# flanggut/smvs

Hardware: NVIDIA H100
Metric: Gauss-Newton Mpix-iters/sec (higher is better)
Workload: dtype f64

## Files before the change

### smvs_b200/csrc/cg.cu

```cuda
#include <algorithm>
#include <cstring>

#include "common.cuh"

namespace smvsb {

namespace {

constexpr int CG_THREADS = 256;
constexpr int CG_WARPS = CG_THREADS / 32;
constexpr int CG_QUADS = CG_THREADS / 4;
constexpr int CG_MAX_BLOCKS = 1024;
constexpr int CG_UF = 4;
constexpr int CG_SLOTS = 10;

struct CgView
{
    int n_nodes, npx;
    int grid;
    int pad;
    double err_tol;
    double const* H;
    double const* P;
    double const* g;
    uint16_t const* rowmask;
    uint32_t const* rows;
    unsigned long long const* counts;
    double* x;
    double* r;
    double* d;
    double* d2;
    double* Ad;
    double* z;
    double* partials;
    double* result;
};

struct CgArgs
{
    int n_views;
    int max_iter;
    double q_tol;
    unsigned int* sync;
    CgView v[SMVSB_MAX_BATCH];
};

struct CgState
{
    double r_dot_r, Q0, beta, alpha, tol;
    double* partials;
    int n_rows, passes, done, iters, info;
    int grid;
};

__device__ __forceinline__ void
grid_barrier (unsigned int* counter, unsigned int& epoch)
{
    __syncthreads();
    if (threadIdx.x == 0)
    {
        epoch += 1;
        unsigned int const target = epoch * gridDim.x;
        asm volatile("red.release.gpu.global.add.u32 [%0], 1;"
            :: "l"(counter) : "memory");
        unsigned int v;
        do {
            asm volatile("ld.relaxed.gpu.global.u32 %0, [%1];"
                : "=r"(v) : "l"(counter) : "memory");
        } while (v < target);
        asm volatile("ld.acquire.gpu.global.u32 %0, [%1];"
            : "=r"(v) : "l"(counter) : "memory");
    }
    __syncthreads();
}

__device__ __forceinline__ unsigned long long
policy_evict_first (void)
{
    unsigned long long pol;
    asm("createpolicy.fractional.L2::evict_first.b64 %0, 1.0;" : "=l"(pol));
    return pol;
}

__device__ __forceinline__ void
ld_stream (double const* p, double2& h01, double2& h23)
{
    unsigned long long const pol = policy_evict_first();
    asm volatile("ld.global.L1::no_allocate.L2::cache_hint.v2.f64 "
        "{%0, %1}, [%2], %3;"
        : "=d"(h01.x), "=d"(h01.y) : "l"(p), "l"(pol));
    asm volatile("ld.global.L1::no_allocate.L2::cache_hint.v2.f64 "
        "{%0, %1}, [%2], %3;"
        : "=d"(h23.x), "=d"(h23.y) : "l"(p + 2), "l"(pol));
}

__device__ __forceinline__ double2
ld_vec (double const* p)
{
    return *reinterpret_cast<double2 const*>(p);
}

__device__ __forceinline__ double2
ld_hint (double const* p, unsigned long long policy)
{
    double2 v;
    asm volatile("ld.global.L2::cache_hint.v2.f64 {%0, %1}, [%2], %3;"
        : "=d"(v.x), "=d"(v.y) : "l"(p), "l"(policy));
    return v;
}

__device__ __forceinline__ unsigned long long
policy_evict_last (void)
{
    unsigned long long pol;
    asm volatile("createpolicy.fractional.L2::evict_last.b64 %0, 1.0;"
        : "=l"(pol));
    return pol;
}

template <int NV>
__device__ __forceinline__ void
warp_flush (double (&v)[NV], double* s_red, int view)
{
#pragma unroll
    for (int j = 0; j < NV; ++j)
        for (int off = 16; off > 0; off >>= 1)
            v[j] += __shfl_down_sync(0xffffffffu, v[j], off);
    if ((threadIdx.x & 31) == 0)
    {
#pragma unroll
        for (int j = 0; j < NV; ++j)
            s_red[(view * 3 + j) * CG_WARPS + (threadIdx.x >> 5)] = v[j];
    }
}

template <int NV>
__device__ __forceinline__ void
publish (CgArgs const& a, CgState const* s_state, double const* s_red,
    int first_slot, bool init)
{
    __syncthreads();
    int const t = threadIdx.x;
    if (t < a.n_views * NV)
    {
        int const view = t / NV, j = t % NV;
        CgState const& S = s_state[view];
        if (static_cast<int>(blockIdx.x) < S.grid && (init || !S.done))
        {
            double total = 0.0;
            if (S.passes > 0)
                for (int i = 0; i < CG_WARPS; ++i)
                    total += s_red[(view * 3 + j) * CG_WARPS + i];
            S.partials[(first_slot + j) * CG_MAX_BLOCKS + blockIdx.x] = total;
        }
    }
}

template <int NV>
__device__ __forceinline__ void
all_sums (CgArgs const& a, CgState const* s_state, int first_slot,
    double* s_bcast, bool init)
{
    __syncthreads();
    int const warp = threadIdx.x >> 5, lane = threadIdx.x & 31;
    for (int pair = warp; pair < a.n_views * NV; pair += CG_WARPS)
    {
        int const view = pair / NV, j = pair % NV;
        if (!init && s_state[view].done)
            continue;
        double const* p = s_state[view].partials
            + (first_slot + j) * CG_MAX_BLOCKS;
        int const nb = s_state[view].grid;
        double v = 0.0;
        for (int base = lane; base < nb; base += 32 * 12)
        {
            double t[12];
#pragma unroll
            for (int u = 0; u < 12; ++u)
                t[u] = (base + 32 * u < nb) ? __ldcg(p + base + 32 * u) : 0.0;
#pragma unroll
            for (int u = 0; u < 12; ++u)
                if (base + 32 * u < nb)
                    v += t[u];
        }
        for (int off = 16; off > 0; off >>= 1)
            v += __shfl_down_sync(0xffffffffu, v, off);
        if (lane == 0)
            s_bcast[view * 3 + j] = v;
    }
    __syncthreads();
}

struct PlainVec
{
    double const* v;
    __device__ __forceinline__ void load (int node, double* out) const
    {
        double2 const a = *reinterpret_cast<double2 const*>(
            v + static_cast<size_t>(node) * 4);
        double2 const b = *reinterpret_cast<double2 const*>(
            v + static_cast<size_t>(node) * 4 + 2);
        out[0] = a.x; out[1] = a.y; out[2] = b.x; out[3] = b.y;
    }
};

struct DirVec
{
    double const* z;
    double const* d_old;
    double beta;
    __device__ __forceinline__ void load (int node, double* out) const
    {
        double2 const z0 = ld_vec(z + static_cast<size_t>(node) * 4);
        double2 const z1 = ld_vec(z + static_cast<size_t>(node) * 4 + 2);
        double2 const d0 = ld_vec(d_old + static_cast<size_t>(node) * 4);
        double2 const d1 = ld_vec(d_old + static_cast<size_t>(node) * 4 + 2);
        out[0] = z0.x + d0.x * beta; out[1] = z0.y + d0.y * beta;
        out[2] = z1.x + d1.x * beta; out[3] = z1.y + d1.y * beta;
    }
};

template <typename VecOp>
__device__ __forceinline__ double
spmv_row (double const* __restrict__ H, int ns, VecOp const& vec, int node,
    int rp, unsigned int mask, double* own)
{
    int const ix = node % ns, iy = node / ns;
    double const* hrow = H + static_cast<size_t>(node) * 144 + rp * 4;
    double acc = 0.0;
    own[0] = 0.0; own[1] = 0.0; own[2] = 0.0; own[3] = 0.0;
    if (mask == 0)
        return 0.0;
#pragma unroll
    for (int k = 0; k < 9; ++k)
    {
        if (!((mask >> k) & 1u))
            continue;
        int const jx = ix + (k % 3) - 1, jy = iy + (k / 3) - 1;
        int const nj = jy * ns + jx;
        double2 h01, h23;
        ld_stream(hrow + k * 16, h01, h23);
        double v[4];
        vec.load(nj, v);
        if (k == 4)
        {
            own[0] = v[0]; own[1] = v[1]; own[2] = v[2]; own[3] = v[3];
        }
        acc += h01.x * v[0];
        acc += h01.y * v[1];
        acc += h23.x * v[2];
        acc += h23.y * v[3];
    }
    return acc;
}

__device__ __forceinline__ bool
view_on (CgArgs const& a, CgState const* s_state, int v, bool init)
{
    return static_cast<int>(blockIdx.x) < s_state[v].grid
        && (init || !s_state[v].done) && s_state[v].passes > 0;
}

__device__ __forceinline__ bool
pass_row (CgView const& V, int n_rows, int pass, int& node)
{
    int const q = pass * (V.grid * CG_QUADS) + blockIdx.x * CG_QUADS
        + (threadIdx.x >> 2);
    bool const ok = q < n_rows;
    node = ok ? static_cast<int>(V.rows[q]) : 0;
    return ok;
}

template <int NV>
__global__ void __launch_bounds__(CG_THREADS, 2)
cg_kernel (CgArgs const a)
{
    unsigned long long const keep = policy_evict_last();
    __shared__ double s_red[NV * 3 * CG_WARPS];
    __shared__ double s_bcast[NV * 3];
    __shared__ CgState s_state[NV];
    __shared__ double const* s_zptr[NV];
    unsigned int epoch = 0;
    int const quad = threadIdx.x & 28;
    int const rp = threadIdx.x & 3;

    if (threadIdx.x < a.n_views)
    {
        CgView const& V = a.v[threadIdx.x];
        CgState& S = s_state[threadIdx.x];
        S.n_rows = static_cast<int>(V.counts[1]);
        int const per_pass = V.grid * CG_QUADS;
        int const passes = (S.n_rows + per_pass - 1) / per_pass;
        S.passes = ((passes + CG_UF - 1) / CG_UF) * CG_UF;
        S.done = 0; S.iters = 0; S.info = SMVSB_CG_MAX_ITERATIONS;
        S.r_dot_r = 0.0; S.Q0 = 0.0; S.beta = 0.0; S.alpha = 0.0; S.tol = 0.0;
        S.partials = V.partials;
        S.grid = V.grid;
        s_zptr[threadIdx.x] = V.z;
    }
    __syncthreads();

#pragma unroll
    for (int v = 0; v < NV; ++v)
    {
        if (v >= a.n_views || !view_on(a, s_state, v, true))
            continue;
        CgView const& V = a.v[v];
        int const n_rows = s_state[v].n_rows, passes = s_state[v].passes;
        double acc[2] = { 0.0, 0.0 };
        for (int p = 0; p < passes; ++p)
        {
            int node;
            bool const ok = pass_row(V, n_rows, p, node);
            size_t const i = static_cast<size_t>(node) * 4 + rp;
            double const gi = ok ? V.g[i] : 0.0;
            double const ri = -gi;
            double const r0 = __shfl_sync(0xffffffffu, ri, quad);
            double const r1 = __shfl_sync(0xffffffffu, ri, quad + 1);
            double const r2 = __shfl_sync(0xffffffffu, ri, quad + 2);
            double const r3 = __shfl_sync(0xffffffffu, ri, quad + 3);
            if (ok)
            {
                double const* prow = V.P + static_cast<size_t>(node) * 16
                    + rp * 4;
                double2 const p01 = *reinterpret_cast<double2 const*>(prow);
                double2 const p23 = *reinterpret_cast<double2 const*>(prow + 2);
                double const zi = p01.x * r0 + p01.y * r1 + p23.x * r2
                    + p23.y * r3;
                V.r[i] = ri;
                V.z[i] = zi;
                V.d[i] = 0.0;
                V.d2[i] = 0.0;
                V.Ad[i] = 0.0;
                acc[1] += gi * gi;
                acc[0] += zi * ri;
            }
        }
        warp_flush<2>(acc, s_red, v);
    }
    publish<2>(a, s_state, s_red, 0, true);
    grid_barrier(a.sync, epoch);
    all_sums<2>(a, s_state, 0, s_bcast, true);
    if (threadIdx.x < a.n_views)
    {
        CgState& S = s_state[threadIdx.x];
        S.r_dot_r = s_bcast[threadIdx.x * 3 + 0];
        double const gg = s_bcast[threadIdx.x * 3 + 1];
        double const et = a.v[threadIdx.x].err_tol;
        S.tol = (et < 0.0) ? sqrt(gg) * 0.01 : et;
    }
    __syncthreads();

    int iter = 1;
    int first_node[NV];
    unsigned int first_mask[NV];
#pragma unroll
    for (int v = 0; v < NV; ++v)
    {
        first_node[v] = 0;
        first_mask[v] = 0u;
        if (v < a.n_views && static_cast<int>(blockIdx.x) < s_state[v].grid)
        {
            int const quad0 = blockIdx.x * CG_QUADS + (threadIdx.x >> 2);
            if (quad0 < s_state[v].n_rows)
            {
                first_node[v] = static_cast<int>(a.v[v].rows[quad0]);
                first_mask[v] = a.v[v].rowmask[first_node[v]];
            }
        }
    }
    for (; iter < a.max_iter; ++iter)
    {
        bool const odd = (iter & 1) != 0;
        int const slot = 2 + 4 * (iter & 1);

        {
#pragma unroll
            for (int v = 0; v < NV; ++v)
            {
                if (v >= a.n_views || !view_on(a, s_state, v, false))
                    continue;
                CgView const& V = a.v[v];
                int const n_rows = s_state[v].n_rows;
                int const quads = V.grid * CG_QUADS;
                int const quad0 = blockIdx.x * CG_QUADS + (threadIdx.x >> 2);
                DirVec dir;
                dir.z = s_zptr[v];
                dir.d_old = odd ? V.d : V.d2;
                dir.beta = s_state[v].beta;
                double* d_new = odd ? V.d2 : V.d;
                double acc[1] = { 0.0 };
                int node = first_node[v];
                unsigned int mask = first_mask[v];
                for (int q = quad0; q < n_rows; q += quads)
                {
                    int const qn = q + quads;
                    int const node_next = (qn < n_rows)
                        ? static_cast<int>(V.rows[qn]) : 0;
                    unsigned int const mask_next = (qn < n_rows)
                        ? V.rowmask[node_next] : 0u;
                    double own[4];
                    size_t const i = static_cast<size_t>(node) * 4 + rp;
                    double const val = spmv_row(V.H, V.npx + 1, dir, node, rp,
                        mask, own);
                    node = node_next;
                    mask = mask_next;
                    double const di = (rp == 0) ? own[0] : (rp == 1) ? own[1]
                        : (rp == 2) ? own[2] : own[3];
                    V.Ad[i] = val;
                    d_new[i] = di;
                    acc[0] += val * di;
                }
                warp_flush<1>(acc, s_red, v);
            }
            publish<1>(a, s_state, s_red, slot, false);
        }
        grid_barrier(a.sync, epoch);
        all_sums<1>(a, s_state, slot, s_bcast, false);
        if (threadIdx.x < a.n_views && !s_state[threadIdx.x].done)
            s_state[threadIdx.x].alpha = s_state[threadIdx.x].r_dot_r
                / s_bcast[threadIdx.x * 3];
        __syncthreads();

#pragma unroll
        for (int v = 0; v < NV; ++v)
        {
            if (v >= a.n_views || !view_on(a, s_state, v, false))
                continue;
            CgView const& V = a.v[v];
            int const n_rows = s_state[v].n_rows;
            int const passes = s_state[v].passes;
            double const alpha = s_state[v].alpha;
            double const* d_new = odd ? V.d2 : V.d;
            double acc[3] = { 0.0, 0.0, 0.0 };
            int nodes[CG_UF];
            bool oks[CG_UF];
#pragma unroll
            for (int u = 0; u < CG_UF; ++u)
                oks[u] = pass_row(V, n_rows, u, nodes[u]);
            for (int p = 0; p < passes; p += CG_UF)
            {
                int nodes_next[CG_UF];
                bool oks_next[CG_UF];
#pragma unroll
                for (int u = 0; u < CG_UF; ++u)
                    oks_next[u] = pass_row(V, n_rows, p + CG_UF + u,
                        nodes_next[u]);

                double xv[CG_UF], rv[CG_UF], gv[CG_UF];
                double2 p01[CG_UF], p23[CG_UF];
#pragma unroll
                for (int u = 0; u < CG_UF; ++u)
                {
                    xv[u] = 0.0; rv[u] = 0.0; gv[u] = 0.0;
                    p01[u] = make_double2(0, 0); p23[u] = p01[u];
                    if (oks[u])
                    {
                        size_t const i = static_cast<size_t>(nodes[u]) * 4 + rp;
                        double const dn = d_new[i], ad = V.Ad[i];
                        gv[u] = V.g[i];
                        xv[u] = V.x[i]; rv[u] = V.r[i];
                        double const* prow = V.P
                            + static_cast<size_t>(nodes[u]) * 16 + rp * 4;
                        p01[u] = ld_hint(prow, keep);
                        p23[u] = ld_hint(prow + 2, keep);
                        xv[u] += dn * alpha; rv[u] -= ad * alpha;
                    }
                }
#pragma unroll
                for (int u = 0; u < CG_UF; ++u)
                {
                    double const q0 = __shfl_sync(0xffffffffu, rv[u], quad);
                    double const q1 = __shfl_sync(0xffffffffu, rv[u], quad + 1);
                    double const q2 = __shfl_sync(0xffffffffu, rv[u], quad + 2);
                    double const q3 = __shfl_sync(0xffffffffu, rv[u], quad + 3);
                    if (oks[u])
                    {
                        size_t const i = static_cast<size_t>(nodes[u]) * 4 + rp;
                        double const zi = p01[u].x * q0 + p01[u].y * q1
                            + p23[u].x * q2 + p23[u].y * q3;
                        V.x[i] = xv[u]; V.r[i] = rv[u];
                        V.z[i] = zi;
                        acc[0] += rv[u] * rv[u];
                        acc[1] += xv[u] * (rv[u] - gv[u]);
                        acc[2] += zi * rv[u];
                    }
                }
#pragma unroll
                for (int u = 0; u < CG_UF; ++u)
                {
                    nodes[u] = nodes_next[u];
                    oks[u] = oks_next[u];
                }
            }
            warp_flush<3>(acc, s_red, v);
        }
        publish<3>(a, s_state, s_red, slot + 1, false);
        grid_barrier(a.sync, epoch);
        all_sums<3>(a, s_state, slot + 1, s_bcast, false);

        if (threadIdx.x < a.n_views && !s_state[threadIdx.x].done)
        {
            CgState& S = s_state[threadIdx.x];
            double const new_rr = s_bcast[threadIdx.x * 3 + 0];
            double const xbr = s_bcast[threadIdx.x * 3 + 1];
            double const new_zr = s_bcast[threadIdx.x * 3 + 2];
            bool stop = false;
            if (new_rr < S.tol)
                stop = true;
            else
            {
                double const Q1 = -1.0 * xbr;
                double const zeta = iter * (Q1 - S.Q0) / Q1;
                if (zeta < a.q_tol)
                    stop = true;
                else
                {
                    S.Q0 = Q1;
                    S.beta = new_zr / S.r_dot_r;
                    S.r_dot_r = new_zr;
                }
            }
            if (stop)
            {
                S.done = 1;
                S.iters = iter;
                S.info = SMVSB_CG_CONVERGENCE;
            }
        }
        __syncthreads();
        bool all_done = true;
        for (int v = 0; v < a.n_views; ++v)
            all_done = all_done && (s_state[v].done != 0);
        if (all_done)
            break;
    }

    if (blockIdx.x == 0 && threadIdx.x < a.n_views)
    {
        CgState const& S = s_state[threadIdx.x];
        double* res = a.v[threadIdx.x].result;
        res[0] = S.done ? S.iters : iter;
        res[1] = S.info;
        res[2] = isnan(__ldcg(a.v[threadIdx.x].x)) ? 1.0 : 0.0;
    }
}

__global__ void __launch_bounds__(256)
cg_mark_kernel (int npx, int npy, uint8_t const* __restrict__ node_valid,
    uint8_t const* __restrict__ active, uint16_t* __restrict__ rowmask,
    uint32_t* __restrict__ block_rows, unsigned long long* __restrict__ counts)
{
    int const node = blockIdx.x * blockDim.x + threadIdx.x;
    int const ns = npx + 1;
    unsigned int m = 0;
    if (node < ns * (npy + 1) && node_valid[node] && active[node])
    {
        int const ix = node % ns, iy = node / ns;
        for (int k = 0; k < 9; ++k)
        {
            int const jx = ix + (k % 3) - 1, jy = iy + (k / 3) - 1;
            if (jx < 0 || jx > npx || jy < 0 || jy > npy)
                continue;
            int const nj = jy * ns + jx;
            if (node_valid[nj] && active[nj])
                m |= 1u << k;
        }
    }
    if (node < ns * (npy + 1))
        rowmask[node] = static_cast<uint16_t>(m);
    unsigned int const blocks = __reduce_add_sync(0xffffffffu, __popc(m));
    int const rows = __syncthreads_count(m != 0);
    if ((threadIdx.x & 31) == 0)
        atomicAdd(counts, static_cast<unsigned long long>(blocks));
    if (threadIdx.x == 0)
    {
        block_rows[blockIdx.x] = rows;
        atomicAdd(counts + 1, static_cast<unsigned long long>(rows));
    }
}

__global__ void __launch_bounds__(1024)
cg_scan_kernel (uint32_t const* __restrict__ block_rows,
    uint32_t* __restrict__ block_off, int nb)
{
    __shared__ uint32_t s_warp[32];
    __shared__ uint32_t s_carry;
    if (threadIdx.x == 0)
        s_carry = 0;
    __syncthreads();
    int const lane = threadIdx.x & 31, warp = threadIdx.x >> 5;
    for (int base = 0; base < nb; base += 1024)
    {
        int const i = base + threadIdx.x;
        uint32_t const v = (i < nb) ? block_rows[i] : 0;
        uint32_t inc = v;
        for (int o = 1; o < 32; o <<= 1)
        {
            uint32_t const u = __shfl_up_sync(0xffffffffu, inc, o);
            if (lane >= o)
                inc += u;
        }
        if (lane == 31)
            s_warp[warp] = inc;
        __syncthreads();
        if (warp == 0)
        {
            uint32_t w = s_warp[lane];
            for (int o = 1; o < 32; o <<= 1)
            {
                uint32_t const u = __shfl_up_sync(0xffffffffu, w, o);
                if (lane >= o)
                    w += u;
            }
            s_warp[lane] = w;
        }
        __syncthreads();
        uint32_t const before = s_carry + (warp > 0 ? s_warp[warp - 1] : 0)
            + inc - v;
        if (i < nb)
            block_off[i] = before;
        __syncthreads();
        if (threadIdx.x == 1023)
            s_carry = before + v;
        __syncthreads();
    }
}

__global__ void __launch_bounds__(256)
cg_list_kernel (int n_nodes, uint16_t const* __restrict__ rowmask,
    uint32_t const* __restrict__ block_off, uint32_t* __restrict__ rows)
{
    __shared__ uint32_t s_warp[8];
    int const node = blockIdx.x * blockDim.x + threadIdx.x;
    bool const on = node < n_nodes && rowmask[node] != 0;
    unsigned int const ballot = __ballot_sync(0xffffffffu, on);
    int const lane = threadIdx.x & 31, warp = threadIdx.x >> 5;
    if (lane == 0)
        s_warp[warp] = __popc(ballot);
    __syncthreads();
    uint32_t before = block_off[blockIdx.x];
    for (int w = 0; w < warp; ++w)
        before += s_warp[w];
    before += __popc(ballot & ((1u << lane) - 1u));
    if (on)
        rows[before] = node;
}

__global__ void
spmv_kernel (int n_nodes, int npx, double const* __restrict__ H,
    uint16_t const* __restrict__ rowmask, double const* __restrict__ x,
    double* __restrict__ y)
{
    int const i = blockIdx.x * blockDim.x + threadIdx.x;
    if (i >= n_nodes * 4)
        return;
    PlainVec vec;
    vec.v = x;
    double own[4];
    y[i] = spmv_row(H, npx + 1, vec, i >> 2, i & 3, rowmask[i >> 2], own);
}

void
mark_system (smvsb_ctx* c)
{
    int const nb = (c->n_nodes + 255) / 256;
    c->cg_rowmask.reserve(c->n_nodes);
    c->cg_row_list.reserve(c->n_nodes);
    c->cg_block_rows.reserve(2 * static_cast<size_t>(nb));
    c->cg_counts.reserve(2);
    CUDA_CHECK(cudaMemsetAsync(c->cg_counts.p, 0,
        2 * sizeof(unsigned long long), c->stream));
    cg_mark_kernel<<<nb, 256, 0, c->stream>>>(c->npx, c->npy,
        c->node_valid.p, c->active.p, c->cg_rowmask.p, c->cg_block_rows.p,
        c->cg_counts.p);
    cg_scan_kernel<<<1, 1024, 0, c->stream>>>(c->cg_block_rows.p,
        c->cg_block_rows.p + nb, nb);
    cg_list_kernel<<<nb, 256, 0, c->stream>>>(c->n_nodes, c->cg_rowmask.p,
        c->cg_block_rows.p + nb, c->cg_row_list.p);
    smvsb::count_launches(c, 3);
    CUDA_CHECK(cudaGetLastError());
}

}

void
launch_spmv (smvsb_ctx* c, double const* x, double* y)
{
    mark_system(c);
    int const n = c->n_nodes * 4;
    spmv_kernel<<<(n + 255) / 256, 256, 0, c->stream>>>(c->n_nodes, c->npx,
        c->H.p, c->cg_rowmask.p, x, y);
    smvsb::count_launches(c, 1);
    CUDA_CHECK(cudaGetLastError());
}

void
cg_enqueue (smvsb_ctx* const* cs, int n, int max_iter, double err_tol,
    double q_tol)
{
    if (n < 1 || n > SMVSB_MAX_BATCH)
        throw Error(SMVSB_ERR_INVALID, "batch size out of range");
    smvsb_ctx* lead = cs[0];
    void const* kernel = nullptr;
    if (n == 1)
        kernel = (void const*)cg_kernel<1>;
    else if (n == 2)
        kernel = (void const*)cg_kernel<2>;
    else if (n <= 4)
        kernel = (void const*)cg_kernel<4>;
    else
        kernel = (void const*)cg_kernel<8>;

    int per_sm = 0;
    CUDA_CHECK(cudaOccupancyMaxActiveBlocksPerMultiprocessor(&per_sm,
        kernel, CG_THREADS, 0));
    if (per_sm < 1)
        throw Error(SMVSB_ERR_CUDA, "cg_kernel does not fit on an SM");
    int const grid_max = std::min(lead->num_sms * std::min(per_sm, 2),
        CG_MAX_BLOCKS);

    CgArgs a;
    a.n_views = n; a.max_iter = max_iter; a.q_tol = q_tol;
    lead->cg_sync.reserve(1);
    a.sync = lead->cg_sync.p;
    int grid = 1;
    for (int k = 0; k < n; ++k)
    {
        smvsb_ctx* c = cs[k];
        size_t const nn = static_cast<size_t>(c->n_nodes) * 4;
        c->x.reserve(nn); c->r.reserve(nn); c->d.reserve(nn);
        c->d2.reserve(nn); c->Ad.reserve(nn); c->z.reserve(nn);
        c->cg_partials.reserve(static_cast<size_t>(CG_SLOTS) * CG_MAX_BLOCKS);
        c->cg_result.reserve(16);
        mark_system(c);
        CUDA_CHECK(cudaMemsetAsync(c->x.p, 0, nn * sizeof(double),
            c->stream));
        CgView& V = a.v[k];
        V.n_nodes = c->n_nodes; V.npx = c->npx; V.pad = 0;
        int const need = static_cast<int>((nn + CG_THREADS - 1) / CG_THREADS);
        V.grid = std::max(1, std::min(grid_max, need));
        grid = std::max(grid, V.grid);
        V.err_tol = err_tol;
        V.H = c->H.p; V.P = c->P.p; V.g = c->g.p;
        V.rowmask = c->cg_rowmask.p; V.rows = c->cg_row_list.p;
        V.counts = c->cg_counts.p;
        V.x = c->x.p; V.r = c->r.p; V.d = c->d.p; V.d2 = c->d2.p;
        V.Ad = c->Ad.p; V.z = c->z.p;
        V.partials = c->cg_partials.p; V.result = c->cg_result.p;
    }
    CUDA_CHECK(cudaMemsetAsync(a.sync, 0, sizeof(unsigned int), lead->stream));
    void* params[] = { &a };
    CUDA_CHECK(cudaLaunchCooperativeKernel(kernel, dim3(grid),
        dim3(CG_THREADS), params, 0, lead->stream));
    smvsb::count_launches(lead, 1);
    CUDA_CHECK(cudaGetLastError());
    for (int k = 0; k < n; ++k)
    {
        smvsb_ctx* c = cs[k];
        CUDA_CHECK(cudaMemcpyAsync(c->h_scalars, c->cg_result.p,
            3 * sizeof(double), cudaMemcpyDeviceToHost, c->stream));
        CUDA_CHECK(cudaMemcpyAsync(c->h_scalars + 8, c->cg_counts.p,
            2 * sizeof(unsigned long long), cudaMemcpyDeviceToHost,
            c->stream));
    }
}

void
cg_collect (smvsb_ctx* c, int* iters, int* info, bool* x0_nan)
{
    double const* res = c->h_scalars;
    unsigned long long counts[2];
    std::memcpy(counts, c->h_scalars + 8, sizeof(counts));
    c->cg_blocks = counts[0];
    c->cg_rows = counts[1];
    if (iters) *iters = static_cast<int>(res[0]);
    if (info) *info = static_cast<int>(res[1]);
    if (x0_nan) *x0_nan = (res[2] != 0.0);
}

void
run_cg (smvsb_ctx* c, int max_iter, double err_tol, double q_tol, int* iters,
    int* info, bool* x0_nan)
{
    smvsb_ctx* cs[1] = { c };
    cg_enqueue(cs, 1, max_iter, err_tol, q_tol);
    CUDA_CHECK(cudaStreamSynchronize(c->stream));
    cg_collect(c, iters, info, x0_nan);
}

}
```

Before: 124.1.

## Pin first-pass Hessian rows in shared memory via bulk async copy

For single-view CG, each block copies the Hessian rows of its first pass of quads into dynamic shared memory once, using TMA bulk copies tracked by an mbarrier. Every CG iteration then reads those rows from shared memory instead of streaming them from global memory, and only later passes still stream. The goal is to cut repeated HBM traffic for H across iterations. In exchange it uses about 75 KB of shared memory per block, adjusts the carveout, and fails outright if two CTAs per SM no longer fit.

Result: faster. 138.1, median of 6 (+11.3%).

```diff
diff --git a/smvs_b200/csrc/cg.cu b/smvs_b200/csrc/cg.cu
--- a/smvs_b200/csrc/cg.cu
+++ b/smvs_b200/csrc/cg.cu
@@ -220,13 +220,45 @@
     }
 };
 
-template <typename VecOp>
+struct StreamRows
+{
+    double const* H;
+    __device__ __forceinline__ double const* row (int node, int rp) const
+    {
+        return H + static_cast<size_t>(node) * 144 + rp * 4;
+    }
+    __device__ __forceinline__ void load (double const* p, double2& h01,
+        double2& h23) const
+    {
+        ld_stream(p, h01, h23);
+    }
+};
+
+constexpr int CG_PIN_STRIDE = 146;
+constexpr size_t CG_PIN_BYTES = sizeof(double) * CG_PIN_STRIDE * CG_QUADS;
+
+struct PinnedRows
+{
+    double const* s;
+    __device__ __forceinline__ double const* row (int, int rp) const
+    {
+        return s + (threadIdx.x >> 2) * CG_PIN_STRIDE + rp * 4;
+    }
+    __device__ __forceinline__ void load (double const* p, double2& h01,
+        double2& h23) const
+    {
+        h01 = *reinterpret_cast<double2 const*>(p);
+        h23 = *reinterpret_cast<double2 const*>(p + 2);
+    }
+};
+
+template <typename Rows, typename VecOp>
 __device__ __forceinline__ double
-spmv_row (double const* __restrict__ H, int ns, VecOp const& vec, int node,
-    int rp, unsigned int mask, double* own)
+spmv_row (Rows const& H, int ns, VecOp const& vec, int node, int rp,
+    unsigned int mask, double* own)
 {
     int const ix = node % ns, iy = node / ns;
-    double const* hrow = H + static_cast<size_t>(node) * 144 + rp * 4;
+    double const* hrow = H.row(node, rp);
     double acc = 0.0;
     own[0] = 0.0; own[1] = 0.0; own[2] = 0.0; own[3] = 0.0;
     if (mask == 0)
@@ -239,7 +271,7 @@
         int const jx = ix + (k % 3) - 1, jy = iy + (k / 3) - 1;
         int const nj = jy * ns + jx;
         double2 h01, h23;
-        ld_stream(hrow + k * 16, h01, h23);
+        H.load(hrow + k * 16, h01, h23);
         double v[4];
         vec.load(nj, v);
         if (k == 4)
@@ -280,9 +312,13 @@
     __shared__ double s_bcast[NV * 3];
     __shared__ CgState s_state[NV];
     __shared__ double const* s_zptr[NV];
+    extern __shared__ __align__(16) double s_pin[];
+    __shared__ __align__(8) unsigned long long s_pin_bar;
     unsigned int epoch = 0;
     int const quad = threadIdx.x & 28;
     int const rp = threadIdx.x & 3;
+    unsigned const pin_bar = static_cast<unsigned>(
+        __cvta_generic_to_shared(&s_pin_bar));
 
     if (threadIdx.x < a.n_views)
     {
@@ -297,8 +333,40 @@
         S.partials = V.partials;
         S.grid = V.grid;
         s_zptr[threadIdx.x] = V.z;
+        if (NV == 1)
+        {
+            int const n_pin = static_cast<int>(blockIdx.x) < V.grid
+                ? min(max(S.n_rows - static_cast<int>(blockIdx.x) * CG_QUADS,
+                  0), CG_QUADS) : 0;
+            if (n_pin > 0)
+            {
+                asm volatile("mbarrier.init.shared::cta.b64 [%0], %1;"
+                    :: "r"(pin_bar), "r"(n_pin));
+                asm volatile("fence.mbarrier_init.release.cluster;"
+                    ::: "memory");
+            }
+        }
     }
     __syncthreads();
+
+    bool const pin = NV == 1 && static_cast<int>(blockIdx.x) < s_state[0].grid
+        && static_cast<int>(blockIdx.x) * CG_QUADS < s_state[0].n_rows;
+    if (NV == 1 && rp == 0)
+    {
+        int node;
+        if (static_cast<int>(blockIdx.x) < s_state[0].grid
+            && pass_row(a.v[0], s_state[0].n_rows, 0, node))
+        {
+            unsigned const dst = static_cast<unsigned>(__cvta_generic_to_shared(
+                s_pin + (threadIdx.x >> 2) * CG_PIN_STRIDE));
+            double const* src = a.v[0].H + static_cast<size_t>(node) * 144;
+            asm volatile("mbarrier.arrive.expect_tx.shared::cta.b64 _, [%0], "
+                "%1;" :: "r"(pin_bar), "r"(1152) : "memory");
+            asm volatile("cp.async.bulk.shared::cluster.global"
+                ".mbarrier::complete_tx::bytes [%0], [%1], %2, [%3];"
+                :: "r"(dst), "l"(src), "r"(1152), "r"(pin_bar) : "memory");
+        }
+    }
 
 #pragma unroll
     for (int v = 0; v < NV; ++v)
@@ -369,6 +437,15 @@
             }
         }
     }
+    if (pin)
+    {
+        unsigned done = 0;
+        while (!done)
+            asm volatile("{\n.reg .pred p;\n"
+                "mbarrier.try_wait.parity.shared::cta.b64 p, [%1], 0;\n"
+                "selp.u32 %0, 1, 0, p;\n}"
+                : "=r"(done) : "r"(pin_bar) : "memory");
+    }
     for (; iter < a.max_iter; ++iter)
     {
         bool const odd = (iter & 1) != 0;
@@ -392,7 +469,7 @@
                 double acc[1] = { 0.0 };
                 int node = first_node[v];
                 unsigned int mask = first_mask[v];
-                for (int q = quad0; q < n_rows; q += quads)
+                auto row_pass = [&](auto const& rows, int q)
                 {
                     int const qn = q + quads;
                     int const node_next = (qn < n_rows)
@@ -401,7 +478,7 @@
                         ? V.rowmask[node_next] : 0u;
                     double own[4];
                     size_t const i = static_cast<size_t>(node) * 4 + rp;
-                    double const val = spmv_row(V.H, V.npx + 1, dir, node, rp,
+                    double const val = spmv_row(rows, V.npx + 1, dir, node, rp,
                         mask, own);
                     node = node_next;
                     mask = mask_next;
@@ -410,7 +487,15 @@
                     V.Ad[i] = val;
                     d_new[i] = di;
                     acc[0] += val * di;
+                };
+                int q = quad0;
+                if (NV == 1 && q < n_rows)
+                {
+                    row_pass(PinnedRows{ s_pin }, q);
+                    q += quads;
                 }
+                for (; q < n_rows; q += quads)
+                    row_pass(StreamRows{ V.H }, q);
                 warp_flush<1>(acc, s_red, v);
             }
             publish<1>(a, s_state, s_red, slot, false);
@@ -657,8 +742,9 @@
         return;
     PlainVec vec;
     vec.v = x;
+    StreamRows const rows{ H };
     double own[4];
-    y[i] = spmv_row(H, npx + 1, vec, i >> 2, i & 3, rowmask[i >> 2], own);
+    y[i] = spmv_row(rows, npx + 1, vec, i >> 2, i & 3, rowmask[i >> 2], own);
 }
 
 void
@@ -712,11 +798,33 @@
     else
         kernel = (void const*)cg_kernel<8>;
 
+    size_t const dyn_smem = (n == 1) ? CG_PIN_BYTES : 0;
+    if (n == 1)
+    {
+        cudaFuncAttributes fa;
+        CUDA_CHECK(cudaFuncGetAttributes(&fa, kernel));
+        int smem_sm = 0, reserved = 0;
+        CUDA_CHECK(cudaDeviceGetAttribute(&smem_sm,
+            cudaDevAttrMaxSharedMemoryPerMultiprocessor, lead->device));
+        CUDA_CHECK(cudaDeviceGetAttribute(&reserved,
+            cudaDevAttrReservedSharedMemoryPerBlock, lead->device));
+        size_t const need = 2 * (dyn_smem + fa.sharedSizeBytes + reserved);
+        int const carveout = static_cast<int>(std::min<size_t>(100,
+            (100 * need + smem_sm - 1) / smem_sm));
+        CUDA_CHECK(cudaFuncSetAttribute(kernel,
+            cudaFuncAttributeMaxDynamicSharedMemorySize,
+            static_cast<int>(dyn_smem)));
+        CUDA_CHECK(cudaFuncSetAttribute(kernel,
+            cudaFuncAttributePreferredSharedMemoryCarveout, carveout));
+    }
     int per_sm = 0;
     CUDA_CHECK(cudaOccupancyMaxActiveBlocksPerMultiprocessor(&per_sm,
-        kernel, CG_THREADS, 0));
+        kernel, CG_THREADS, dyn_smem));
     if (per_sm < 1)
         throw Error(SMVSB_ERR_CUDA, "cg_kernel does not fit on an SM");
+    if (n == 1 && per_sm < 2)
+        throw Error(SMVSB_ERR_CUDA, "cg_kernel<1> fits only "
+            + std::to_string(per_sm) + " CTA per SM, needs 2");
     int const grid_max = std::min(lead->num_sms * std::min(per_sm, 2),
         CG_MAX_BLOCKS);
 
@@ -752,7 +860,7 @@
     CUDA_CHECK(cudaMemsetAsync(a.sync, 0, sizeof(unsigned int), lead->stream));
     void* params[] = { &a };
     CUDA_CHECK(cudaLaunchCooperativeKernel(kernel, dim3(grid),
-        dim3(CG_THREADS), params, 0, lead->stream));
+        dim3(CG_THREADS), params, dyn_smem, lead->stream));
     smvsb::count_launches(lead, 1);
     CUDA_CHECK(cudaGetLastError());
     for (int k = 0; k < n; ++k)
```
